# pps-lab/rofl-project-code

Measured on AMD Instinct MI355X. Metric: range-proof elements/sec (create+verify), d=25k 32-bit, higher is better.
Workload: dtype u32x8 (255-bit integer field)

## Files before the change

### rofl_project_code_amd/csrc/host_prover.hpp

```cpp
#pragma once

void tr_append_point(Merlin &t, const char *label, const ge5 &p, uint8_t *enc_out) {
    uint8_t e[32]; h51::encode(e, p); t.append(label, e, 32); if (enc_out) memcpy(enc_out, e, 32);
}
void fill_pow2(sc *tab, sc base_mont, int count) { tab[0] = base_mont; for (int i = 1; i < count; i++) tab[i] = sc_montmul(tab[i - 1], tab[i - 1]); }

sc sum_partials(const sc *p, size_t count, size_t stride, size_t which) {
    sc acc = sc_zero();
    for (size_t i = 0; i < count; i++) acc = sc_add(acc, p[i * stride + which]);
    return acc;
}

struct ChunkNonce { int mode; NonceSeed seed; const uint8_t *d_stream; u64 stream_scalars, base; };
void prove_chunks(Ctx &C, const char *label, size_t P, size_t n, size_t m, const u64 *d_vshift, const sc *d_blind,
                  const std::vector<ChunkNonce> &nonces, const uint8_t *h_V , uint8_t *const *proofs_out,
                  hipEvent_t v_ready = nullptr ) {
    size_t N = n * m; unsigned lgN = lg2u(N);
    static const bool ptrace = knob("ROFL_TRACE") && atoi(knob("ROFL_TRACE")) >= 2;
    double pt0 = now_ms(), ptl = pt0;
    auto mark = [&](const char *what, long a = -1) {
        if (!ptrace) return;
        double t = now_ms(); fprintf(stderr, "[rofl-trace lane=%p] %-14s %6ld  +%.3f ms  (t=%.3f)\n", (void *)&C, what, a, t - ptl, t - pt0); ptl = t;
    };
    size_t plen = 32 * (9 + 2 * (size_t)lgN);
    GensPin gens = get_gens(C, n, m);
    niels *tbl = gens.tbl();
    const niels *wtab = gens.wtab();
    ChunkParams *h_cp = C.h_cp.as<ChunkParams>(P);
    ChunkParams *d_cp = C.cp.as<ChunkParams>(P);
    memset(h_cp, 0, sizeof(ChunkParams) * P);
    u64 per = (u64)m * (2 * n + 4);
    for (size_t c = 0; c < P; c++) {
        h_cp[c].nonce_base = nonces[c].base; h_cp[c].nonce_mode = nonces[c].mode; h_cp[c].nonce_seed = nonces[c].seed;
        h_cp[c].nonce_stream = nonces[c].d_stream; h_cp[c].nonce_stream_scalars = nonces[c].stream_scalars;
    }
    HIPCHK(hipMemcpyAsync(d_cp, h_cp, sizeof(ChunkParams) * P, hipMemcpyHostToDevice, C.stream));
    sc *sL = C.sL.as<sc>(P * N), *sR = C.sR.as<sc>(P * N), *party = C.party.as<sc>(P * 4 * m), *Scanon = C.Scanon.as<sc>(P * 2 * N);
    ROFL_LAUNCH(k_nonce_expand, grid1(per / 2 + 1, (u32)P), dim3(TPB), 0, C.stream, (u32)n, (u32)m, d_cp, sL, sR, party, Scanon);
    if (!C.stream2) HIPCHK(hipStreamCreateWithFlags(&C.stream2, hipStreamNonBlocking));
    if (!C.ev_a) { HIPCHK(hipEventCreateWithFlags(&C.ev_a, hipEventDisableTiming)); HIPCHK(hipEventCreateWithFlags(&C.ev_a0, hipEventDisableTiming)); }
    HIPCHK(hipEventRecord(C.ev_a0, C.stream));
    HIPCHK(hipStreamWaitEvent(C.stream2, C.ev_a0, 0));
    ge *partial = C.partial.as<ge>(P * m);
    ROFL_LAUNCH(k_bitcommit, grid1(m, (u32)P), dim3(TPB), 0, C.stream2, (u32)n, (u32)m, d_vshift, tbl, partial);
    u32 nblkA = (u32)std::min<size_t>(16, (m + TPB - 1) / TPB);
    ge *partial2 = C.partial2.as<ge>(P * nblkA);
    ROFL_LAUNCH(k_point_sum, dim3(nblkA, (u32)P), dim3(TPB), TPB * sizeof(ge), C.stream2, partial, (u32)m, partial2);
    ge *h_A = C.h_part.as<ge>(P * nblkA);
    HIPCHK(hipMemcpyAsync(h_A, partial2, sizeof(ge) * P * nblkA, hipMemcpyDeviceToHost, C.stream2));
    HIPCHK(hipEventRecord(C.ev_a, C.stream2));
    u32 nblkS = (u32)std::min<size_t>(16, (m + TPB - 1) / TPB);
    sc *scpart = C.scpart.as<sc>(P * 64 * 3);
    PowTabs *d_pt = C.powtabs.as<PowTabs>(P);
    ROFL_LAUNCH(k_party_sums, dim3(nblkS, (u32)P), dim3(TPB), 0, C.stream, (u32)m, 0, d_cp, (const PowTabs *)d_pt, party, d_blind, scpart);
    sc *h_sc = C.h_misc2.as<sc>(P * 64 * 3);
    HIPCHK(hipMemcpyAsync(h_sc, scpart, sizeof(sc) * P * nblkS * 3, hipMemcpyDeviceToHost, C.stream));
    std::vector<MsmProb> probs(P); std::vector<ge5> res;
    for (size_t c = 0; c < P; c++) probs[c] = MsmProb{tbl, Scanon + c * 2 * N};
    C.tm.t.msm_terms += P * 2 * N;
    mark("setup");
    std::vector<Merlin> tr; tr.reserve(P);
    std::vector<sc> a_bl(P), s_bl(P), y(P), z(P), zz(P), x(P), w(P);
    for (size_t c = 0; c < P; c++) tr.emplace_back(label, strlen(label));
    {
        MsmOpt mo; mo.tag = 99; if (wtab) { gens.fb_for(P, &mo.fb_wtab, &mo.fb_c); mo.fb_stride = 2 * N; }
        mo.overlap = [&]() {
            double t0 = now_ms();
            if (v_ready) HIPCHK(hipEventSynchronize(v_ready));
            C.pool->run(P, [&](size_t c) {
                Merlin &t = tr[c];
                t.append("dom-sep", (const uint8_t *)"rangeproof v1", 13);
                t.append_u64("n", n); t.append_u64("m", m);
                t.append32_run('V', h_V + c * m * 32, m);
            });
            C.tm.t.host_ms += now_ms() - t0;
        };
        msm_run(C, probs, 2 * N, res, mo);
    }
    mark("msm S");
    HIPCHK(hipEventSynchronize(C.ev_a));

    double th = now_ms();
    C.pool->run(P, [&](size_t c) {
        uint8_t *o = proofs_out[c];
        Merlin &t = tr[c];
        a_bl[c] = h_canon(sum_partials(h_sc + c * nblkS * 3, nblkS, 3, 0));
        s_bl[c] = h_canon(sum_partials(h_sc + c * nblkS * 3, nblkS, 3, 1));
        ge5 A = h_fixed_mul(C.ht.Bb5, a_bl[c]);
        for (u32 k = 0; k < nblkA; k++) A = h51::gadd(A, h51::from_ge(h_A[c * nblkA + k]));
        ge5 S = h51::gadd(res[c], h_fixed_mul(C.ht.Bb5, s_bl[c]));
        tr_append_point(t, "A", A, o); tr_append_point(t, "S", S, o + 32);
        y[c] = t.challenge_scalar("y"); z[c] = t.challenge_scalar("z");
        zz[c] = h_mul(z[c], z[c]);
        ChunkParams &cp = h_cp[c];
        cp.y = h_mont(y[c]); cp.z = h_mont(z[c]); cp.zz = h_mont(zz[c]);
        cp.yinv = h_mont(h_inv(y[c]));
        fill_pow2(cp.ypow2, cp.y, MAX_LG); fill_pow2(cp.yinvpow2, cp.yinv, MAX_LG); fill_pow2(cp.zpow2, cp.z, MAX_LG);
    });
    C.tm.t.host_ms += now_ms() - th;
    mark("y z host");
    HIPCHK(hipMemcpyAsync(d_cp, h_cp, sizeof(ChunkParams) * P, hipMemcpyHostToDevice, C.stream));
    u32 nblkT = (u32)std::min<size_t>(std::max<size_t>(64, std::min<size_t>(256, 2048 / P)), (N + TPB - 1) / TPB);
    sc *tpart = C.tmp_out.as<sc>(P * 256 * 3);
    ROFL_LAUNCH(k_pow_tables, dim3((4 * PT_L * PT_E + TPB - 1) / TPB, (u32)P), dim3(TPB), 0, C.stream, d_cp, d_pt, lgN, 0);
    ROFL_LAUNCH(k_poly_t, dim3(nblkT, (u32)P), dim3(TPB), 0, C.stream, (u32)n, (u32)m, d_cp, (const PowTabs *)d_pt, d_vshift, sL, sR, C.d_two_pow, tpart);
    ROFL_LAUNCH(k_party_sums, dim3(nblkS, (u32)P), dim3(TPB), 0, C.stream, (u32)m, 1, d_cp, (const PowTabs *)d_pt, party, d_blind, scpart);
    sc *h_t = C.h_part.as<sc>(P * 256 * 3);
    HIPCHK(hipMemcpyAsync(h_t, tpart, sizeof(sc) * P * nblkT * 3, hipMemcpyDeviceToHost, C.stream));
    HIPCHK(hipMemcpyAsync(h_sc, scpart, sizeof(sc) * P * nblkS * 3, hipMemcpyDeviceToHost, C.stream));
    C.sync();
    mark("t kernels");
    th = now_ms();
    C.pool->run(P, [&](size_t c) {
        uint8_t *o = proofs_out[c];
        Merlin &t = tr[c];
        sc t0 = h_canon(sum_partials(h_t + c * nblkT * 3, nblkT, 3, 0));
        sc t1 = h_canon(sum_partials(h_t + c * nblkT * 3, nblkT, 3, 1));
        sc t2 = h_canon(sum_partials(h_t + c * nblkT * 3, nblkT, 3, 2));
        sc t1_bl = h_canon(sum_partials(h_sc + c * nblkS * 3, nblkS, 3, 0));
        sc t2_bl = h_canon(sum_partials(h_sc + c * nblkS * 3, nblkS, 3, 1));
        sc zvbl = h_canon(sum_partials(h_sc + c * nblkS * 3, nblkS, 3, 2));
        ge5 T1 = h51::gadd(h_fixed_mul(C.ht.B5, t1), h_fixed_mul(C.ht.Bb5, t1_bl));
        ge5 T2 = h51::gadd(h_fixed_mul(C.ht.B5, t2), h_fixed_mul(C.ht.Bb5, t2_bl));
        tr_append_point(t, "T_1", T1, o + 64); tr_append_point(t, "T_2", T2, o + 96);
        x[c] = t.challenge_scalar("x");
        sc xx = h_mul(x[c], x[c]);
        sc t_x = sc_add(sc_add(t0, h_mul(t1, x[c])), h_mul(t2, xx));
        sc t_x_bl = sc_add(sc_add(zvbl, h_mul(t1_bl, x[c])), h_mul(t2_bl, xx));
        sc e_bl = sc_add(a_bl[c], h_mul(s_bl[c], x[c]));
        t.append_scalar("t_x", t_x); t.append_scalar("t_x_blinding", t_x_bl); t.append_scalar("e_blinding", e_bl);
        sc_tobytes(o + 128, t_x); sc_tobytes(o + 160, t_x_bl); sc_tobytes(o + 192, e_bl);
        w[c] = t.challenge_scalar("w");
        h_cp[c].x = h_mont(x[c]);
        h_cp[c].gscale = sc_one_mont(); h_cp[c].hscale = sc_one_mont();
        t.append("dom-sep", (const uint8_t *)"ipp v1", 6);
        t.append_u64("n", N);
    });
    C.tm.t.host_ms += now_ms() - th;
    mark("T x host");
    HIPCHK(hipMemcpyAsync(d_cp, h_cp, sizeof(ChunkParams) * P, hipMemcpyHostToDevice, C.stream));
    sc *a = C.a.as<sc>(P * N), *b = C.b.as<sc>(P * N), *yinvpow = C.yinv.as<sc>(P * N);
    const u32 lr_first_blocks = (u32)std::min<size_t>(256, (N / 2 + TPB - 1) / TPB);
    ROFL_LAUNCH(k_lr_first, dim3(lr_first_blocks, (u32)P), dim3(TPB), 0, C.stream, (u32)n, (u32)m, d_cp, (const PowTabs *)d_pt, d_vshift, sL, sR, C.d_two_pow, a, b, yinvpow,
                       C.SL.as<sc>(P * 2 * N), C.h_ip.dev<sc>(P * 256 * 2));
    mark("poly/T/x");

    size_t n_g = N; unsigned r = 0;
    std::vector<const niels *> cur(P, tbl);
    std::vector<std::vector<sc>> pu(P), pui(P);
    std::vector<sc> gscale(P, sc_one_mont()), hscale(P, sc_one_mont());
    int gsel = 0; bool first_level = true;
    auto stab = [&](size_t c, u32 h, sc &g, sc &hh) {
        g = sc_one_mont(); hh = sc_one_mont();
        for (unsigned q = 0; q < r; q++) {
            bool bit = (h >> (r - 1 - q)) & 1;
            g = sc_montmul(g, bit ? pu[c][q] : pui[c][q]);
            hh = sc_montmul(hh, bit ? pui[c][q] : pu[c][q]);
        }
    };
    sc *h_round = C.h_round.as<sc>(2 * P);
    sc *a2 = C.a2.as<sc>(P * N), *b2 = C.b2.as<sc>(P * N);
    bool just_materialised = false;
    sc *ptab[2] = {C.ptab[0].as<sc>(P * 2 * N), C.ptab[1].as<sc>(P * 2 * N)}; int psel = 0;
    std::unique_ptr<std::atomic<int>[]> lr_done(new std::atomic<int>[P]);
    sc *ip_dev = C.ipdev.as<sc>(P * 256 * 2);
    niels *d_q = C.qpts.as<niels>(P);
    {
        niels *h_q = C.h_q.as<niels>(P);
        C.pool->run(P, [&](size_t c) { h_q[c] = h51::to_niels32(h_fixed_mul(C.ht.B5, w[c])); });
        HIPCHK(hipMemcpyAsync(d_q, h_q, sizeof(niels) * P, hipMemcpyHostToDevice, C.stream));
    }
    bool ip_included = false, pts_pending = false;
    std::vector<ge5> cq;
    for (unsigned round = 0; round < lgN; round++) {
        size_t n_k = n_g >> r, nh = n_k / 2;
        sc *SL = C.SL.as<sc>(P * 2 * n_g);
        u32 nblkI = lr_first_blocks;
        sc *h_ip = C.h_ip.as<sc>(P * 256 * 2);
        if (round > 0) {
            nblkI = (u32)std::min<size_t>(256, std::max<size_t>(1, (n_g + TPB - 1) / TPB));
            int use_new = just_materialised ? 0 : 1;
            ROFL_LAUNCH(k_ipp_round, dim3(nblkI, (u32)P), dim3(TPB), 0, C.stream, (u32)n_g, (u32)n_k, use_new ? r - 1 : 0u, use_new, d_cp,
                               (const sc *)C.h_round.dev<sc>(2 * P), (const sc *)a, (const sc *)b, a2, b2, N, yinvpow, N, SL, C.h_ip.dev<sc>(P * 256 * 2),
                               (const sc *)ptab[psel], ptab[psel ^ 1], N, n_k == 2 ? C.h_abfin.dev<sc>(4 * P) : (sc *)nullptr, ip_dev);
            std::swap(a, a2); std::swap(b, b2); psel ^= 1;
        }
        just_materialised = false;
        if (!C.ev_ip) HIPCHK(hipEventCreateWithFlags(&C.ev_ip, hipEventDisableTiming));
        HIPCHK(hipEventRecord(C.ev_ip, C.stream));
        std::vector<MsmProb> pr(2 * P);
        for (size_t c = 0; c < P; c++) { pr[2 * c] = MsmProb{cur[c], SL + c * 2 * n_g}; pr[2 * c + 1] = MsmProb{cur[c], SL + c * 2 * n_g}; }
        C.tm.t.msm_terms += P * 2 * n_g;
        MsmOpt mo;
        mo.lr_nh = (u32)nh; mo.lr_ng = (u32)n_g;
        mo.tag = 100 + round;
        if (pts_pending) { mo.pts_ready = C.ev_norm; pts_pending = false; }
        if (round > 0) { mo.ip_dev = ip_dev; mo.ip_nblk = nblkI; mo.qpts = d_q; mo.ip_included = &ip_included; }
        if (first_level && wtab) { gens.fb_for(2 * P, &mo.fb_wtab, &mo.fb_c); mo.fb_stride = 2 * N; }
        for (size_t c = 0; c < P; c++) lr_done[c].store(0);
        bool cq_ready = false;
        auto cq_of = [&](size_t p) { sc cx = h_canon(sum_partials(h_ip + (p >> 1) * nblkI * 2, nblkI, 2, p & 1)); return h_fixed_mul(C.ht.B5, h_mul(cx, w[p >> 1])); };
        mo.overlap = [&]() {
            if (ip_included) return;
            C.wait_event(C.ev_ip);
            cq.resize(2 * P);
            C.pool->run(2 * P, [&](size_t p) { cq[p] = cq_of(p); });
            cq_ready = true;
        };
        auto with_cq = [&](size_t p) { return ip_included ? res[p] : h51::gadd(res[p], cq_ready ? cq[p] : cq_of(p)); };
        mo.post = [&](size_t p) {
            size_t c = p >> 1; int side = (int)(p & 1);
            uint8_t *o = proofs_out[c] + 7 * 32 + 64 * round;
            h51::encode(o + 32 * side, with_cq(p));
            if (lr_done[c].fetch_add(1) != 1) return;
            tr[c].append("L", o, 32); tr[c].append("R", o + 32, 32);
            sc u = tr[c].challenge_scalar("u");
            sc um = h_mont(u), uim = h51::sc_invert_mont_fast(um);
            h_round[2 * c] = um; h_round[2 * c + 1] = uim;
            h_cp[c].pend_u[pu[c].size()] = um; h_cp[c].pend_ui[pu[c].size()] = uim;
            pu[c].push_back(um); pui[c].push_back(uim);
        };
        mo.post8 = [&](size_t p0, int cnt) {
            ge5 pts[8];
            for (int l = 0; l < 8; l++) {
                if (l >= cnt) { pts[l] = h51::identity(); continue; }
                pts[l] = with_cq(p0 + (size_t)l);
            }
            uint8_t enc[8][32];
            h8::encode8(enc, pts);
            const int nch = cnt / 2;
            sc um[4], pre[4];
            for (int k = 0; k < nch; k++) {
                size_t c = (p0 >> 1) + (size_t)k;
                uint8_t *o = proofs_out[c] + 7 * 32 + 64 * round;
                memcpy(o, enc[2 * k], 32); memcpy(o + 32, enc[2 * k + 1], 32);
                tr[c].append("L", o, 32); tr[c].append("R", o + 32, 32);
                um[k] = h_mont(tr[c].challenge_scalar("u"));
                pre[k] = k ? sc_montmul(pre[k - 1], um[k]) : um[k];
            }
            sc uim[4];
            if (nch && !sc_iszero(h_canon(pre[nch - 1]))) {
                sc inv = h51::sc_invert_mont_fast(pre[nch - 1]);
                for (int k = nch - 1; k >= 1; k--) { uim[k] = sc_montmul(inv, pre[k - 1]); inv = sc_montmul(inv, um[k]); }
                uim[0] = inv;
            } else
                for (int k = 0; k < nch; k++) uim[k] = h51::sc_invert_mont_fast(um[k]);
            for (int k = 0; k < nch; k++) {
                size_t c = (p0 >> 1) + (size_t)k;
                h_round[2 * c] = um[k]; h_round[2 * c + 1] = uim[k];
                h_cp[c].pend_u[pu[c].size()] = um[k]; h_cp[c].pend_ui[pu[c].size()] = uim[k];
                pu[c].push_back(um[k]); pui[c].push_back(uim[k]);
            }
        };
        msm_run(C, pr, 2 * n_g, res, mo);
        mark("round msm", (long)(2 * n_g));
        bool last = (round + 1 == lgN);
        r++;
        unsigned t_now = first_level ? (unsigned)C.fold_t1 : (unsigned)C.fold_t;
        size_t n_after = n_g >> r;
        bool fold_pays = n_after >= C.fold_min || (n_after >= 64 && 2 * P * n_after >= 8 * C.fold_min);
        if (!last && r >= t_now && fold_pays) {
            size_t n_new = n_g >> r; u32 nsrc = 1u << r;
            bool use_tab = first_level && C.fold_tab;
            FoldTabCfg fc = gens.fc();
            size_t dstride = use_tab ? (size_t)fc.np * FOLD_TAB_DIGITS : 256;
            th = now_ms();
            const size_t dbytes = use_tab ? 2 : 1;
            int8_t *h_dig = C.h_fdig.as<int8_t>(2 * P * nsrc * dstride * dbytes);
            int16_t *h_dig16 = reinterpret_cast<int16_t *>(h_dig);
            memset(h_dig, 0, 2 * P * nsrc * dstride * dbytes);
            FoldProb *h_fp = C.h_fprob.as<FoldProb>(2 * P);
            niels *gnew = C.gbuf[gsel].as<niels>(P * 2 * n_new);
            std::vector<int> topc(P, 0);
            C.pool->run(P, [&](size_t c) {
                int top = 0;
                sc yn = sc_one_mont();
                sc ystep = sc_one_mont();
                { size_t e = n_new; int bidx = 0; while (e) { if (e & 1) ystep = sc_montmul(ystep, h_cp[c].yinvpow2[bidx]); e >>= 1; bidx++; } }
                sc g0, h0; stab(c, 0, g0, h0);
                sc gall, hall; stab(c, nsrc - 1, gall, hall);
                for (u32 h = 1; h < nsrc; h++) {
                    sc g, hh; stab(c, h, g, hh);
                    yn = sc_montmul(yn, ystep);
                    hh = sc_montmul(hh, yn);
                    g = sc_montmul(g, gall); hh = sc_montmul(hh, hall);
                    sc gc = h_canon(g), hc = h_canon(hh);
                    if (use_tab) {
                        for (u32 pc = 0; pc < fc.np; pc++) {
                            auto piece = [&](const sc &s) {
                                u32 bit0 = pc * fc.pb; u64 lo = (u64)s.v[bit0 / 32] | ((bit0 / 32 + 1 < 8) ? (u64)s.v[bit0 / 32 + 1] << 32 : 0);
                                lo >>= (bit0 % 32);
                                return fc.pb == 64 ? lo : (lo & (((u64)1 << fc.pb) - 1));
                            };
                            int t1 = wnaf_u64(h_dig16 + (((2 * c) * nsrc + h) * fc.np + pc) * FOLD_TAB_DIGITS, piece(gc), fc.w);
                            int t2 = wnaf_u64(h_dig16 + (((2 * c + 1) * nsrc + h) * fc.np + pc) * FOLD_TAB_DIGITS, piece(hc), fc.w);
// ... 117 lines not shown
```

### rofl_project_code_amd/csrc/kernels.hpp

```cpp
#pragma once
#include <type_traits>
#include "fe32.hpp"
#include "fe26.hpp"
#include "quad26.hpp"
#include "keccak.hpp"

namespace rofl {

#define TPB 256

#ifndef ROFL_KGROUP
#define ROFL_KGROUP 0
#endif
#define ROFL_KG(g) (ROFL_KGROUP == 0 || ROFL_KGROUP == (g))

typedef unsigned int v4u __attribute__((ext_vector_type(4)));
typedef __attribute__((address_space(1))) v4u g_uint4;
__device__ __forceinline__ niels gload_niels(const niels *p) {
    niels r;
    const g_uint4 *s = (const g_uint4 *)p;
    v4u *d = reinterpret_cast<v4u *>(&r);
#pragma unroll
    for (int i = 0; i < 6; i++) d[i] = s[i];
    return r;
// ... 285 lines not shown
    if (v != v) st |= 2;
    if (st) { atomicOr(status, st); vshift[i] = 0; return; }
    double x = fabs((double)v) * (double)(1ULL << fp_frac);
    double lim = ldexp(1.0, (int)fp_bits);
    u64 maxbits = fp_bits >= 64 ? ~0ULL : ((1ULL << fp_bits) - 1);
    u64 k;
    if (x >= lim) k = maxbits;
    else { double r = rint(x); k = (r >= lim) ? maxbits : (u64)r; }
    u64 off = 1ULL << (prove_range - 1);
    u64 lowbits;
    if (v < 0.0f) {
        if (off >= k) lowbits = off - k;
        else {
            u64 l_lo = ((u64)SC_L1 << 32) | SC_L0;
            lowbits = l_lo - (k - off);
        }
    } else lowbits = k + off;
    vshift[i] = lowbits & maxbits;
}
#endif

__device__ __forceinline__ gd fixed_base_mul_acc(gd acc, const niels *tab, const sc &k, int nwin) {
    int carry = 0;
    for (int i = 0; i < nwin; i++) {
        int v = (int)((k.v[i >> 2] >> ((i & 3) * 8)) & 255) + carry;
        carry = (v + 128) >> 8;
        int dgt = v - (carry << 8);
        int ad = dgt < 0 ? -dgt : dgt;
        if (ad) acc = gd_madd(acc, load_nd(&tab[i * 128 + ad - 1]), dgt < 0);
    }
    if (carry && nwin < 32) acc = gd_madd(acc, load_nd(&tab[nwin * 128 + 0]), false);
    return acc;
}
#if ROFL_KG(4)
__global__ void __launch_bounds__(TPB) k_commit(u32 count, const u64 *v64, const sc *v256_canon, const sc *blind_canon ,
                         const niels *tabB, const niels *tabBb, const niels *shift ,
                         uint8_t *V_out , uint8_t *C_out , u32 c_count, u32 c_period) {
    u32 j = blockIdx.x * blockDim.x + threadIdx.x;
    if (j >= count) return;
    gd acc = gd_identity();
    if (v64) { sc v = sc_from_u64(v64[j]); acc = fixed_base_mul_acc(acc, tabB, v, 8); }
    else { sc v = load_sc_reduced(&v256_canon[j]); acc = fixed_base_mul_acc(acc, tabB, v, 32); }
    if (blind_canon) { sc r = load_sc_reduced(&blind_canon[j]); acc = fixed_base_mul_acc(acc, tabBb, r, 32); }
    if (V_out) gd_ristretto_encode(V_out + (size_t)j * 32, acc);
    if (C_out && (j % c_period) < c_count) {
        gd cpt = shift ? gd_madd(acc, load_nd(shift), false) : acc;
        gd_ristretto_encode(C_out + (size_t)j * 32, cpt);
    }
}
#endif

#if ROFL_KG(4)
__global__ void __launch_bounds__(TPB) k_bitcommit(u32 n, u32 m, const u64 *vshift , const niels *tbl, ge *partial ) {
    u32 c = blockIdx.y;
    u32 j = blockIdx.x * blockDim.x + threadIdx.x;
    if (j >= m) return;
    size_t N = (size_t)n * m;
    u64 v = vshift[(size_t)c * m + j];
    gd acc = gd_identity();
    for (u32 i = 0; i < n; i++) {
        bool bit = (v >> i) & 1;
        const niels *p = bit ? &tbl[(size_t)j * n + i] : &tbl[N + (size_t)j * n + i];
        acc = gd_madd(acc, gload_nd(p), !bit);
    }
    store_gd(&partial[(size_t)c * m + j], acc);
}
#endif

#if ROFL_KG(4)
__global__ void __launch_bounds__(TPB) k_point_sum(const ge *in, u32 n, ge *out) {
    extern __shared__ __align__(16) unsigned char smem[];
    ge *lds = reinterpret_cast<ge *>(smem);
    u32 p = blockIdx.y, t = threadIdx.x;
    const ge *src = in + (size_t)p * n;
    ge acc = ge_identity();
    for (u32 i = blockIdx.x * blockDim.x + t; i < n; i += gridDim.x * blockDim.x) acc = ge_add(acc, load_ge(&src[i]));
    lds[t] = acc;
    __syncthreads();
    for (u32 s = blockDim.x / 2; s > 0; s >>= 1) {
        if (t < s) lds[t] = ge_add(lds[t], lds[t + s]);
        __syncthreads();
    }
    if (t == 0) store_ge(&out[(size_t)p * gridDim.x + blockIdx.x], lds[0]);
}
#endif

#if ROFL_KG(4)
__global__ void __launch_bounds__(TPB) k_niels_sum(const niels *in, u32 n, size_t stride, ge *out) {
    extern __shared__ __align__(16) unsigned char smem[];
    ge *lds = reinterpret_cast<ge *>(smem);
    u32 t = threadIdx.x;
    const niels *src = in + (size_t)blockIdx.y * stride;
    gd acc = gd_identity();
    for (u32 i = blockIdx.x * blockDim.x + t; i < n; i += gridDim.x * blockDim.x) acc = gd_madd(acc, load_nd(&src[i]), false);
    lds[t] = gd_pack(acc);
    __syncthreads();
    for (u32 s = blockDim.x / 2; s > 0; s >>= 1) {
        if (t < s) lds[t] = ge_add(lds[t], lds[t + s]);
        __syncthreads();
    }
    if (t == 0) store_ge(&out[(size_t)blockIdx.y * gridDim.x + blockIdx.x], lds[0]);
}
#endif

#if ROFL_KG(4)
__global__ void __launch_bounds__(TPB) k_decode_sum(const uint8_t *in, u32 n, u32 stride, ge *out, u32 *status) {
    extern __shared__ __align__(16) unsigned char smem[];
    ge *lds = reinterpret_cast<ge *>(smem);
    u32 t = threadIdx.x;
    gd gacc = gd_identity();
    for (u32 i = blockIdx.x * blockDim.x + t; i < n; i += gridDim.x * blockDim.x) {
        __align__(16) uint8_t b[32];
        const uint8_t *s = in + (size_t)i * stride;
        for (int q = 0; q < 32; q++) b[q] = s[q];
        gd p;
        if (!gd_ristretto_decode(p, b)) { atomicOr(status, 4u); p = gd_identity(); }
        gacc = gd_add(gacc, p);
    }
    lds[t] = gd_pack(gacc);
    __syncthreads();
    for (u32 s = blockDim.x / 2; s > 0; s >>= 1) {
        if (t < s) lds[t] = ge_add(lds[t], lds[t + s]);
        __syncthreads();
    }
    if (t == 0) store_ge(&out[blockIdx.x], lds[0]);
}
#endif

#if ROFL_KG(4)
__global__ void __launch_bounds__(TPB) k_party_sums(u32 m, int phase, const ChunkParams *cp, const PowTabs *pt, const sc *party, const sc *blind_canon , sc *out) {
    __shared__ sc lds[TPB * 3];
    u32 c = blockIdx.y;
    sc v[3] = {sc_zero(), sc_zero(), sc_zero()};
    for (u32 j = blockIdx.x * blockDim.x + threadIdx.x; j < m; j += gridDim.x * blockDim.x) {
        if (phase == 0) {
            v[0] = sc_add(v[0], load_sc(&party[((size_t)c * 4 + 0) * m + j]));
            v[1] = sc_add(v[1], load_sc(&party[((size_t)c * 4 + 1) * m + j]));
        } else {
            v[0] = sc_add(v[0], load_sc(&party[((size_t)c * 4 + 2) * m + j]));
            v[1] = sc_add(v[1], load_sc(&party[((size_t)c * 4 + 3) * m + j]));
            sc zj = sc_montmul(cp[c].zz, pt_pow(pt[c].z, cp[c].zpow2, j));
            sc bl = sc_to_mont(load_sc(&blind_canon[(size_t)c * m + j]));
            v[2] = sc_add(v[2], sc_montmul(zj, bl));
        }
    }
    block_sum_sc<3>(v, lds);
    if (threadIdx.x == 0) {
#pragma unroll
        for (int k = 0; k < 3; k++) store_sc(&out[((size_t)c * gridDim.x + blockIdx.x) * 3 + k], v[k]);
    }
}
#endif

__device__ __forceinline__ void slot_vectors(const ChunkParams &P, const PowTabs &T, u32 n, u32 k, u64 v, const sc &sR,
                                             sc &l0, sc &r0, sc &r1, const sc *two_pow) {
    u32 j = k / n, i = k % n;
    bool bit = (v >> i) & 1;
    sc one = sc_one_mont();
    sc aL = bit ? one : sc_zero();
    sc aR = bit ? sc_zero() : sc_neg(one);
    sc yk = pt_pow(T.y, P.ypow2, k);
    l0 = sc_sub(aL, P.z);
    sc zj2 = sc_montmul(sc_montmul(P.zz, pt_pow(T.z, P.zpow2, j)), two_pow[i]);
    r0 = sc_add(sc_montmul(yk, sc_add(aR, P.z)), zj2);
    r1 = sc_montmul(yk, sR);
}
#if ROFL_KG(4)
__global__ void __launch_bounds__(TPB) k_poly_t(u32 n, u32 m, const ChunkParams *cp, const PowTabs *pt, const u64 *vshift, const sc *sL, const sc *sR,
                         const sc *two_pow, sc *out) {
    __shared__ sc lds[TPB * 3];
    u32 c = blockIdx.y;
    size_t N = (size_t)n * m;
    sc v[3] = {sc_zero(), sc_zero(), sc_zero()};
    for (u32 k = blockIdx.x * blockDim.x + threadIdx.x; k < N; k += gridDim.x * blockDim.x) {
        sc l0, r0, r1;
        sc l1 = load_sc(&sL[c * N + k]);
        slot_vectors(cp[c], pt[c], n, k, vshift[(size_t)c * m + k / n], load_sc(&sR[c * N + k]), l0, r0, r1, two_pow);
        v[0] = sc_add(v[0], sc_montmul(l0, r0));
        v[1] = sc_add(v[1], sc_add(sc_montmul(l0, r1), sc_montmul(l1, r0)));
        v[2] = sc_add(v[2], sc_montmul(l1, r1));
    }
    block_sum_sc<3>(v, lds);
    if (threadIdx.x == 0) {
#pragma unroll
        for (int k = 0; k < 3; k++) store_sc(&out[((size_t)c * gridDim.x + blockIdx.x) * 3 + k], v[k]);
    }
}
#endif

#if ROFL_KG(4)
__global__ void __launch_bounds__(TPB, 3) k_lr_first(u32 n, u32 m, const ChunkParams *cp, const PowTabs *pt, const u64 *vshift, const sc *sL, const sc *sR,
                           const sc *two_pow, sc *a, sc *b, sc *yinvpow, sc *SL, sc *ip_out) {
    __shared__ sc lds[TPB * 2];
    const u32 c = blockIdx.y;
    const size_t N = (size_t)n * m;
    const u32 nh = (u32)(N / 2);
    const sc sG = load_sc(&cp[c].gscale), sH0 = load_sc(&cp[c].hscale), x = cp[c].x;
    sc *sl = SL + (size_t)c * 2 * N;
    sc v[2] = {sc_zero(), sc_zero()};
    for (u32 i = blockIdx.x * blockDim.x + threadIdx.x; i < nh; i += gridDim.x * blockDim.x) {
        sc a0 = sc_zero(), b0 = a0, y0 = a0, a1 = a0, b1 = a0, y1 = a0;
#pragma unroll 1
        for (int s = 0; s < 2; s++) {
            const u32 k = s ? nh + i : i;
            sc l0, r0, r1;
            sc l1 = load_sc(&sL[c * N + k]);
            slot_vectors(cp[c], pt[c], n, k, vshift[(size_t)c * m + k / n], load_sc(&sR[c * N + k]), l0, r0, r1, two_pow);
            sc ao = sc_add(l0, sc_montmul(l1, x));
            sc bo = sc_add(r0, sc_montmul(r1, x));
            sc yo = pt_pow(pt[c].yinv, cp[c].yinvpow2, k);
            store_sc(&a[c * N + k], ao); store_sc(&b[c * N + k], bo); store_sc(&yinvpow[c * N + k], yo);
            if (s == 0) { a0 = ao; b0 = bo; y0 = yo; } else { a1 = ao; b1 = bo; y1 = yo; }
        }
        store_sc(&sl[i], sc_from_mont(sc_montmul(a1, sG)));
        store_sc(&sl[N + i], sc_from_mont(sc_montmul(b1, sc_montmul(sH0, y0))));
        store_sc(&sl[nh + i], sc_from_mont(sc_montmul(a0, sG)));
        store_sc(&sl[N + nh + i], sc_from_mont(sc_montmul(b0, sc_montmul(sH0, y1))));
        v[0] = sc_add(v[0], sc_montmul(a0, b1));
        v[1] = sc_add(v[1], sc_montmul(a1, b0));
    }
    block_sum_sc<2>(v, lds);
    if (threadIdx.x == 0) {
        store_sc(&ip_out[((size_t)c * gridDim.x + blockIdx.x) * 2 + 0], v[0]);
        store_sc(&ip_out[((size_t)c * gridDim.x + blockIdx.x) * 2 + 1], v[1]);
    }
}
#endif


#if ROFL_KG(4)
__global__ void __launch_bounds__(TPB) k_ipp_round(u32 n_g, u32 n_k, u32 r_prev, int use_new, ChunkParams *cp, const sc *round_ch, const sc *a_in, const sc *b_in,
                                                   sc *a_out, sc *b_out, size_t ab_stride, const sc *yinvpow, size_t y_stride, sc *SL, sc *ip_out,
                                                   const sc *ptab_in, sc *ptab_out, size_t ptab_stride, sc *ab_host, sc *ip_dev) {
    __shared__ sc lds[TPB * 2];
    __shared__ sc s_u[2];
    u32 c = blockIdx.y;
    if (threadIdx.x == 0) { s_u[0] = load_sc(&round_ch[2 * c]); s_u[1] = load_sc(&round_ch[2 * c + 1]); }
    __syncthreads();
    const sc u = s_u[0], ui = s_u[1];
    if (use_new && blockIdx.x == 0 && threadIdx.x == 0) { store_sc(&cp[c].pend_u[r_prev], u); store_sc(&cp[c].pend_ui[r_prev], ui); }
    const sc *ai = a_in + c * ab_stride, *bi = b_in + c * ab_stride;
    sc *ao = a_out + c * ab_stride, *bo = b_out + c * ab_stride;
    const u32 nh = n_k / 2;
    const sc gs = sc_from_mont(load_sc(&cp[c].gscale)), hs = sc_from_mont(load_sc(&cp[c].hscale));
    sc *sl = SL + (size_t)c * 2 * n_g;
    sc v[2] = {sc_zero(), sc_zero()};
    auto fold2 = [](const sc &x, const sc &cu, const sc &y, const sc &cv) {
        u32 w[17];
#pragma unroll
        for (int q = 0; q < 17; q++) w[q] = 0;
        sc_mac_wide(w, x, cu); sc_mac_wide(w, y, cv);
        return sc_redc_wide(w);
    };
    for (u32 j = blockIdx.x * blockDim.x + threadIdx.x; j < n_g; j += gridDim.x * blockDim.x) {
        u32 h = j / n_k, i = j % n_k;
        bool lo = i < nh; u32 ii = lo ? nh + i : i - nh;
        sc af = fold2(load_sc(&ai[ii]), u, load_sc(&ai[n_k + ii]), ui);
        sc bf = fold2(load_sc(&bi[ii]), ui, load_sc(&bi[n_k + ii]), u);
        u32 hp = use_new ? h >> 1 : h;
        sc tG = r_prev ? load_sc(&ptab_in[(size_t)c * 2 * ptab_stride + hp]) : gs;
        sc tH = r_prev ? load_sc(&ptab_in[(size_t)c * 2 * ptab_stride + ptab_stride + hp]) : hs;
        if (use_new) { bool bit = h & 1; tG = sc_montmul(tG, bit ? u : ui); tH = sc_montmul(tH, bit ? ui : u); }
        if (i == 0) { store_sc(&ptab_out[(size_t)c * 2 * ptab_stride + h], tG); store_sc(&ptab_out[(size_t)c * 2 * ptab_stride + ptab_stride + h], tH); }
        const sc sG = tG, sH = sc_montmul(tH, load_sc(&yinvpow[c * y_stride + j]));
        store_sc(&sl[j], sc_montmul(af, sG));
        store_sc(&sl[n_g + j], sc_montmul(bf, sH));
        if (h == 0) {
            store_sc(&ao[ii], af); store_sc(&bo[ii], bf);
            if (ab_host && n_k == 2) { store_sc(&ab_host[c * 4 + ii], af); store_sc(&ab_host[c * 4 + 2 + ii], bf); }
            if (lo) {
                sc al = fold2(load_sc(&ai[i]), u, load_sc(&ai[n_k + i]), ui);
                sc bl = fold2(load_sc(&bi[i]), ui, load_sc(&bi[n_k + i]), u);
                v[0] = sc_add(v[0], sc_montmul(al, bf));
                v[1] = sc_add(v[1], sc_montmul(af, bl));
            }
        }
    }
    block_sum_sc<2>(v, lds);
    if (threadIdx.x == 0) {
        store_sc(&ip_out[((size_t)c * gridDim.x + blockIdx.x) * 2 + 0], v[0]);
        store_sc(&ip_out[((size_t)c * gridDim.x + blockIdx.x) * 2 + 1], v[1]);
        if (ip_dev) {
            store_sc(&ip_dev[((size_t)c * gridDim.x + blockIdx.x) * 2 + 0], v[0]);
            store_sc(&ip_dev[((size_t)c * gridDim.x + blockIdx.x) * 2 + 1], v[1]);
        }
    }
}
#endif

struct FoldProb { const niels *src; niels *dst; };
#define FOLD_MAXSRC 64
#define FOLD_MAXSEG 4
struct FoldSeg { int lo[FOLD_MAXSEG + 1]; };
#if ROFL_KG(2)
__global__ void __launch_bounds__(256, 4) k_fold_gens(u32 n_new, u32 nsrc, FoldSeg seg, const FoldProb *probs, const int8_t *naf , int unit_first) {
    extern __shared__ __align__(16) unsigned char smem[];
    ge *lds = reinterpret_cast<ge *>(smem);
    u32 q = blockIdx.y;
    u32 i = blockIdx.x * 64 + threadIdx.x;
    u32 k = threadIdx.y, K = blockDim.y;
    bool active = i < n_new;
    const niels *src = probs[q].src;
    const int8_t *dg = naf + (size_t)q * nsrc * 256;
    gd acc = gd_identity();
    if (active) {
        int lo = seg.lo[k], hi = seg.lo[k + 1] - 1;
        for (int bit = hi; bit >= lo; bit--) {
            acc = gd_double(acc);
            for (u32 h = unit_first ? 1 : 0; h < nsrc; h++) {
                int d = dg[h * 256 + bit];
                if (d != 0) acc = gd_madd(acc, gload_nd(&src[(size_t)h * n_new + i]), d < 0);
            }
        }
        for (int t = 0; t < lo; t++) acc = gd_double(acc);
    }
    if (K > 1) {
        if (k > 0) lds[(k - 1) * 64 + threadIdx.x] = gd_pack(acc);
        __syncthreads();
        if (k == 0)
            for (u32 s2 = 1; s2 < K; s2++) acc = gd_add(acc, gd_unpack(lds[(s2 - 1) * 64 + threadIdx.x]));
    }
    if (active && k == 0) {
        if (unit_first) acc = gd_madd(acc, gload_nd(&src[i]), false);
        gstore_niels(&probs[q].dst[i], gd_to_niels(acc));
    }
}
#endif

#if ROFL_KG(2)
__global__ void __launch_bounds__(256, 2) k_fold_gens4(u32 n_new, FoldSeg seg, const FoldProb *probs, const int8_t *naf ) {
    extern __shared__ __align__(16) unsigned char smem[];
    ge *lds = reinterpret_cast<ge *>(smem);
    u32 q = blockIdx.y;
    u32 i = blockIdx.x * 64 + threadIdx.x;
    u32 k = threadIdx.y, K = blockDim.y;
    bool active = i < n_new;
    const niels *src = probs[q].src;
    const int8_t *dg = naf + (size_t)q * 4 * 256;
    gd acc = gd_identity();
    if (active) {
        const nd s1 = gload_nd(&src[(size_t)1 * n_new + i]), s2 = gload_nd(&src[(size_t)2 * n_new + i]), s3 = gload_nd(&src[(size_t)3 * n_new + i]);
        int lo = seg.lo[k], hi = seg.lo[k + 1] - 1;
        for (int bit = hi; bit >= lo; bit--) {
            acc = gd_double(acc);
            int d1 = dg[256 + bit], d2 = dg[512 + bit], d3 = dg[768 + bit];
            if (d1 != 0) acc = gd_madd(acc, s1, d1 < 0);
            if (d2 != 0) acc = gd_madd(acc, s2, d2 < 0);
            if (d3 != 0) acc = gd_madd(acc, s3, d3 < 0);
        }
        for (int t = 0; t < lo; t++) acc = gd_double(acc);
    }
    if (K > 1) {
        if (k > 0) lds[(k - 1) * 64 + threadIdx.x] = gd_pack(acc);
        __syncthreads();
        if (k == 0)
            for (u32 s2i = 1; s2i < K; s2i++) acc = gd_add(acc, gd_unpack(lds[(s2i - 1) * 64 + threadIdx.x]));
    }
    if (active && k == 0) {
        acc = gd_madd(acc, gload_nd(&src[i]), false);
        gstore_niels(&probs[q].dst[i], gd_to_niels(acc));
    }
}
#endif

#define FOLD_TAB_DIGITS 72
struct FoldWProb { const niels *src; niels *dst; u32 tab_off, ev_off, n_ev, seg_start[FOLD_MAXSEG]; };
#define FOLD_EV(bit, h, e, neg) ((u32)(bit) | ((u32)(h) << 9) | ((u32)(e) << 15) | ((u32)(neg) << 27))
#if ROFL_KG(2)
__device__ __forceinline__ void fold_w_body(u32 n_new, const FoldSeg &seg, const FoldWProb *probs, const u32 *events, const niels *tab, size_t tstride, ge *ext_out) {
    extern __shared__ __align__(16) unsigned char smem[];
    ge *lds = reinterpret_cast<ge *>(smem);
    const u32 q = blockIdx.y;
    const u32 i = blockIdx.x * 64 + threadIdx.x;
    const u32 k = threadIdx.y, K = blockDim.y;
    const bool active = i < n_new;
    const niels *src = probs[q].src;
    const u32 *ev = events + probs[q].ev_off;
    gd acc = gd_identity();
    if (active) {
        const niels *tb = tab + probs[q].tab_off;
        auto operand = [&](u32 w) { const u32 h = (w >> 9) & 63u, e = (w >> 15) & 4095u;
                                    const niels *p = e ? tb + (size_t)(e - 1) * tstride : src;
                                    return gload_nd(&p[(size_t)h * n_new + i]); };
        const int lo = seg.lo[k];
        int pos = seg.lo[k + 1];
        u32 j = probs[q].seg_start[k];
        const u32 jend = k == 0 ? probs[q].n_ev : probs[q].seg_start[k - 1];
        if (j < jend) {
            u32 w = ev[j];
            nd nxt = operand(w);
            while (j < jend) {
                const nd cur = nxt; const u32 wc = w;
                j++;
                if (j < jend) { w = ev[j]; nxt = operand(w); }
                const int b = (int)(wc & 511u);
                for (; pos > b; pos--) acc = gd_double(acc);
                acc = gd_madd(acc, cur, (wc >> 27) & 1u);
            }
        }
        for (; pos > lo; pos--) acc = gd_double(acc);
        for (int t = 0; t < lo; t++) acc = gd_double(acc);
    }
    if (K > 1) {
        if (k > 0) lds[(k - 1) * 64 + threadIdx.x] = gd_pack(acc);
        __syncthreads();
        if (k == 0)
            for (u32 s2 = 1; s2 < K; s2++) acc = gd_add(acc, gd_unpack(lds[(s2 - 1) * 64 + threadIdx.x]));
    }
    if (active && k == 0) {
        acc = gd_madd(acc, gload_nd(&src[i]), false);
        if (ext_out) store_gd(&ext_out[(size_t)q * n_new + i], acc);
        else gstore_niels(&probs[q].dst[i], gd_to_niels(acc));
    }
}
__global__ void __launch_bounds__(256, 2) k_fold_gens_w(u32 n_new, FoldSeg seg, const FoldWProb *probs, const u32 *events, const niels *tab, size_t tstride, ge *ext_out) {
    fold_w_body(n_new, seg, probs, events, tab, tstride, ext_out);
}
#endif

#define NB_BATCH 8
#if ROFL_KG(2)
__global__ void __launch_bounds__(TPB) k_niels_batch(u32 count, const ge *ext, niels *out) {
    const u32 t = blockIdx.x * blockDim.x + threadIdx.x;
    const size_t i0 = (size_t)t * NB_BATCH;
    if (i0 >= count) return;
    const u32 nb = (u32)min((size_t)NB_BATCH, (size_t)count - i0);
    fe pre[NB_BATCH];
    fd run = fd_unpack(reinterpret_cast<const fe *>(&ext[i0])[2]);
// ... 1554 lines not shown
```

Before: 1.148 million.

## Process slot runs incrementally and hoist per-block pending scales in IPP round

```diff
diff --git a/rofl_project_code_amd/csrc/host_prover.hpp b/rofl_project_code_amd/csrc/host_prover.hpp
--- a/rofl_project_code_amd/csrc/host_prover.hpp
+++ b/rofl_project_code_amd/csrc/host_prover.hpp
@@ -100,7 +100,7 @@
     C.tm.t.host_ms += now_ms() - th;
     mark("y z host");
     HIPCHK(hipMemcpyAsync(d_cp, h_cp, sizeof(ChunkParams) * P, hipMemcpyHostToDevice, C.stream));
-    u32 nblkT = (u32)std::min<size_t>(std::max<size_t>(64, std::min<size_t>(256, 2048 / P)), (N + TPB - 1) / TPB);
+    u32 nblkT = (u32)std::min<size_t>(std::max<size_t>(64, std::min<size_t>(256, 2048 / P)), (N / SLOT_RUN + TPB - 1) / TPB);
     sc *tpart = C.tmp_out.as<sc>(P * 256 * 3);
     ROFL_LAUNCH(k_pow_tables, dim3((4 * PT_L * PT_E + TPB - 1) / TPB, (u32)P), dim3(TPB), 0, C.stream, d_cp, d_pt, lgN, 0);
     ROFL_LAUNCH(k_poly_t, dim3(nblkT, (u32)P), dim3(TPB), 0, C.stream, (u32)n, (u32)m, d_cp, (const PowTabs *)d_pt, d_vshift, sL, sR, C.d_two_pow, tpart);
@@ -140,7 +140,7 @@
     mark("T x host");
     HIPCHK(hipMemcpyAsync(d_cp, h_cp, sizeof(ChunkParams) * P, hipMemcpyHostToDevice, C.stream));
     sc *a = C.a.as<sc>(P * N), *b = C.b.as<sc>(P * N), *yinvpow = C.yinv.as<sc>(P * N);
-    const u32 lr_first_blocks = (u32)std::min<size_t>(256, (N / 2 + TPB - 1) / TPB);
+    const u32 lr_first_blocks = (u32)std::min<size_t>(256, (N / 2 / SLOT_RUN + TPB - 1) / TPB);
     ROFL_LAUNCH(k_lr_first, dim3(lr_first_blocks, (u32)P), dim3(TPB), 0, C.stream, (u32)n, (u32)m, d_cp, (const PowTabs *)d_pt, d_vshift, sL, sR, C.d_two_pow, a, b, yinvpow,
                        C.SL.as<sc>(P * 2 * N), C.h_ip.dev<sc>(P * 256 * 2));
     mark("poly/T/x");
diff --git a/rofl_project_code_amd/csrc/kernels.hpp b/rofl_project_code_amd/csrc/kernels.hpp
--- a/rofl_project_code_amd/csrc/kernels.hpp
+++ b/rofl_project_code_amd/csrc/kernels.hpp
@@ -461,18 +461,25 @@
 }
 #endif
 
-__device__ __forceinline__ void slot_vectors(const ChunkParams &P, const PowTabs &T, u32 n, u32 k, u64 v, const sc &sR,
-                                             sc &l0, sc &r0, sc &r1, const sc *two_pow) {
-    u32 j = k / n, i = k % n;
-    bool bit = (v >> i) & 1;
-    sc one = sc_one_mont();
-    sc aL = bit ? one : sc_zero();
-    sc aR = bit ? sc_zero() : sc_neg(one);
-    sc yk = pt_pow(T.y, P.ypow2, k);
-    l0 = sc_sub(aL, P.z);
-    sc zj2 = sc_montmul(sc_montmul(P.zz, pt_pow(T.z, P.zpow2, j)), two_pow[i]);
-    r0 = sc_add(sc_montmul(yk, sc_add(aR, P.z)), zj2);
+#define SLOT_RUN 4
+struct SlotConsts { sc y, z, zm1, l0_set, l0_clr; };
+__device__ __forceinline__ SlotConsts slot_consts(const ChunkParams &P) {
+    SlotConsts K;
+    K.y = P.y; K.z = P.z;
+    K.l0_clr = sc_neg(P.z);
+    K.l0_set = sc_add(sc_one_mont(), K.l0_clr);
+    K.zm1 = sc_neg(K.l0_set);
+    return K;
+}
+__device__ __forceinline__ sc slot_run_zj2(const ChunkParams &P, const PowTabs &T, u32 n, u32 k0, const sc *two_pow) {
+    return sc_montmul(sc_montmul(P.zz, pt_pow(T.z, P.zpow2, k0 / n)), two_pow[k0 % n]);
+}
+__device__ __forceinline__ void slot_step(const SlotConsts &K, bool bit, const sc &sR, sc &yk, sc &zj2, sc &l0, sc &r0, sc &r1) {
+    l0 = bit ? K.l0_set : K.l0_clr;
+    r0 = sc_add(sc_montmul(yk, bit ? K.z : K.zm1), zj2);
     r1 = sc_montmul(yk, sR);
+    yk = sc_montmul(yk, K.y);
+    zj2 = sc_add(zj2, zj2);
 }
 #if ROFL_KG(4)
 __global__ void __launch_bounds__(TPB) k_poly_t(u32 n, u32 m, const ChunkParams *cp, const PowTabs *pt, const u64 *vshift, const sc *sL, const sc *sR,
@@ -480,15 +487,29 @@
     __shared__ sc lds[TPB * 3];
     u32 c = blockIdx.y;
     size_t N = (size_t)n * m;
+    const u32 runs = (u32)(N / SLOT_RUN);
+    const SlotConsts K = slot_consts(cp[c]);
     sc v[3] = {sc_zero(), sc_zero(), sc_zero()};
-    for (u32 k = blockIdx.x * blockDim.x + threadIdx.x; k < N; k += gridDim.x * blockDim.x) {
-        sc l0, r0, r1;
-        sc l1 = load_sc(&sL[c * N + k]);
-        slot_vectors(cp[c], pt[c], n, k, vshift[(size_t)c * m + k / n], load_sc(&sR[c * N + k]), l0, r0, r1, two_pow);
-        v[0] = sc_add(v[0], sc_montmul(l0, r0));
-        v[1] = sc_add(v[1], sc_add(sc_montmul(l0, r1), sc_montmul(l1, r0)));
-        v[2] = sc_add(v[2], sc_montmul(l1, r1));
-    }
+    sc r0_all = sc_zero(), r0_set = r0_all, r1_all = r0_all, r1_set = r0_all;
+    for (u32 q = blockIdx.x * blockDim.x + threadIdx.x; q < runs; q += gridDim.x * blockDim.x) {
+        const u32 k0 = q * SLOT_RUN;
+        const u64 bits = vshift[(size_t)c * m + k0 / n] >> (k0 % n);
+        sc yk = pt_pow(pt[c].y, cp[c].ypow2, k0);
+        sc zj2 = slot_run_zj2(cp[c], pt[c], n, k0, two_pow);
+#pragma unroll 1
+        for (u32 s = 0; s < SLOT_RUN; s++) {
+            sc l0, r0, r1;
+            sc l1 = load_sc(&sL[c * N + k0 + s]);
+            const bool bit = (bits >> s) & 1;
+            slot_step(K, bit, load_sc(&sR[c * N + k0 + s]), yk, zj2, l0, r0, r1);
+            r0_all = sc_add(r0_all, r0); r0_set = sc_add(r0_set, bit ? r0 : sc_zero());
+            r1_all = sc_add(r1_all, r1); r1_set = sc_add(r1_set, bit ? r1 : sc_zero());
+            v[1] = sc_add(v[1], sc_montmul(l1, r0));
+            v[2] = sc_add(v[2], sc_montmul(l1, r1));
+        }
+    }
+    v[0] = sc_add(r0_set, sc_montmul(K.l0_clr, r0_all));
+    v[1] = sc_add(v[1], sc_add(r1_set, sc_montmul(K.l0_clr, r1_all)));
     block_sum_sc<3>(v, lds);
     if (threadIdx.x == 0) {
 #pragma unroll
@@ -498,35 +519,45 @@
 #endif
 
 #if ROFL_KG(4)
-__global__ void __launch_bounds__(TPB, 3) k_lr_first(u32 n, u32 m, const ChunkParams *cp, const PowTabs *pt, const u64 *vshift, const sc *sL, const sc *sR,
+__global__ void __launch_bounds__(TPB, 2) k_lr_first(u32 n, u32 m, const ChunkParams *cp, const PowTabs *pt, const u64 *vshift, const sc *sL, const sc *sR,
                            const sc *two_pow, sc *a, sc *b, sc *yinvpow, sc *SL, sc *ip_out) {
     __shared__ sc lds[TPB * 2];
     const u32 c = blockIdx.y;
     const size_t N = (size_t)n * m;
-    const u32 nh = (u32)(N / 2);
-    const sc sG = load_sc(&cp[c].gscale), sH0 = load_sc(&cp[c].hscale), x = cp[c].x;
+    const u32 nh = (u32)(N / 2), lgh = 31 - __clz(nh);
+    const SlotConsts K = slot_consts(cp[c]);
+    const sc x = cp[c].x, yinv = cp[c].yinv;
+    const sc gs = sc_from_mont(load_sc(&cp[c].gscale)), hs = sc_from_mont(load_sc(&cp[c].hscale));
     sc *sl = SL + (size_t)c * 2 * N;
     sc v[2] = {sc_zero(), sc_zero()};
-    for (u32 i = blockIdx.x * blockDim.x + threadIdx.x; i < nh; i += gridDim.x * blockDim.x) {
-        sc a0 = sc_zero(), b0 = a0, y0 = a0, a1 = a0, b1 = a0, y1 = a0;
-#pragma unroll 1
-        for (int s = 0; s < 2; s++) {
-            const u32 k = s ? nh + i : i;
+    for (u32 q = blockIdx.x * blockDim.x + threadIdx.x; q < nh / SLOT_RUN; q += gridDim.x * blockDim.x) {
+        const u32 i0 = q * SLOT_RUN;
+        const u64 bits0 = vshift[(size_t)c * m + i0 / n] >> (i0 % n), bits1 = vshift[(size_t)c * m + (nh + i0) / n] >> ((nh + i0) % n);
+        sc yk0 = pt_pow(pt[c].y, cp[c].ypow2, i0), yo0 = pt_pow(pt[c].yinv, cp[c].yinvpow2, i0);
+        sc yk1 = sc_montmul(yk0, load_sc(&cp[c].ypow2[lgh])), yo1 = sc_montmul(yo0, load_sc(&cp[c].yinvpow2[lgh]));
+        sc zj0 = slot_run_zj2(cp[c], pt[c], n, i0, two_pow), zj1 = slot_run_zj2(cp[c], pt[c], n, nh + i0, two_pow);
+        auto half = [&](u32 k, bool bit, sc &yk, sc &zj2, sc &yo, sc &ao, sc &bo) {
             sc l0, r0, r1;
             sc l1 = load_sc(&sL[c * N + k]);
-            slot_vectors(cp[c], pt[c], n, k, vshift[(size_t)c * m + k / n], load_sc(&sR[c * N + k]), l0, r0, r1, two_pow);
-            sc ao = sc_add(l0, sc_montmul(l1, x));
-            sc bo = sc_add(r0, sc_montmul(r1, x));
-            sc yo = pt_pow(pt[c].yinv, cp[c].yinvpow2, k);
+            slot_step(K, bit, load_sc(&sR[c * N + k]), yk, zj2, l0, r0, r1);
+            ao = sc_add(l0, sc_montmul(l1, x));
+            bo = sc_add(r0, sc_montmul(r1, x));
             store_sc(&a[c * N + k], ao); store_sc(&b[c * N + k], bo); store_sc(&yinvpow[c * N + k], yo);
-            if (s == 0) { a0 = ao; b0 = bo; y0 = yo; } else { a1 = ao; b1 = bo; y1 = yo; }
-        }
-        store_sc(&sl[i], sc_from_mont(sc_montmul(a1, sG)));
-        store_sc(&sl[N + i], sc_from_mont(sc_montmul(b1, sc_montmul(sH0, y0))));
-        store_sc(&sl[nh + i], sc_from_mont(sc_montmul(a0, sG)));
-        store_sc(&sl[N + nh + i], sc_from_mont(sc_montmul(b0, sc_montmul(sH0, y1))));
-        v[0] = sc_add(v[0], sc_montmul(a0, b1));
-        v[1] = sc_add(v[1], sc_montmul(a1, b0));
+        };
+#pragma unroll 1
+        for (u32 s = 0; s < SLOT_RUN; s++) {
+            const u32 i = i0 + s;
+            sc a0, b0, a1, b1;
+            half(i, (bits0 >> s) & 1, yk0, zj0, yo0, a0, b0);
+            half(nh + i, (bits1 >> s) & 1, yk1, zj1, yo1, a1, b1);
+            store_sc(&sl[i], sc_montmul(a1, gs));
+            store_sc(&sl[N + i], sc_montmul(b1, sc_montmul(hs, yo0)));
+            store_sc(&sl[nh + i], sc_montmul(a0, gs));
+            store_sc(&sl[N + nh + i], sc_montmul(b0, sc_montmul(hs, yo1)));
+            v[0] = sc_add(v[0], sc_montmul(a0, b1));
+            v[1] = sc_add(v[1], sc_montmul(a1, b0));
+            yo0 = sc_montmul(yo0, yinv); yo1 = sc_montmul(yo1, yinv);
+        }
     }
     block_sum_sc<2>(v, lds);
     if (threadIdx.x == 0) {
@@ -551,7 +582,6 @@
     const sc *ai = a_in + c * ab_stride, *bi = b_in + c * ab_stride;
     sc *ao = a_out + c * ab_stride, *bo = b_out + c * ab_stride;
     const u32 nh = n_k / 2;
-    const sc gs = sc_from_mont(load_sc(&cp[c].gscale)), hs = sc_from_mont(load_sc(&cp[c].hscale));
     sc *sl = SL + (size_t)c * 2 * n_g;
     sc v[2] = {sc_zero(), sc_zero()};
     auto fold2 = [](const sc &x, const sc &cu, const sc &y, const sc &cv) {
@@ -561,28 +591,46 @@
         sc_mac_wide(w, x, cu); sc_mac_wide(w, y, cv);
         return sc_redc_wide(w);
     };
-    for (u32 j = blockIdx.x * blockDim.x + threadIdx.x; j < n_g; j += gridDim.x * blockDim.x) {
+    auto pending = [&](u32 h, u32 side) {
+        sc t = r_prev ? load_sc(&ptab_in[(size_t)c * 2 * ptab_stride + side * ptab_stride + (use_new ? h >> 1 : h)])
+                      : sc_from_mont(load_sc(side ? &cp[c].hscale : &cp[c].gscale));
+        if (use_new) t = sc_montmul(t, ((h & 1) != side) ? u : ui);
+        return t;
+    };
+    const bool block_h = n_k % TPB == 0;
+    __shared__ sc s_t[2];
+    for (u32 j0 = blockIdx.x * blockDim.x; j0 < n_g; j0 += gridDim.x * blockDim.x) {
+        const u32 j = j0 + threadIdx.x;
+        sc tG, tH;
+        if (block_h) {
+            __syncthreads();
+            if (threadIdx.x < 2) {
+                const u32 h0 = j0 / n_k;
+                sc t = pending(h0, threadIdx.x);
+                s_t[threadIdx.x] = t;
+                if (j0 % n_k == 0) store_sc(&ptab_out[(size_t)c * 2 * ptab_stride + threadIdx.x * ptab_stride + h0], t);
+            }
+            __syncthreads();
+            tG = s_t[0]; tH = s_t[1];
+        }
+        if (j >= n_g) continue;
         u32 h = j / n_k, i = j % n_k;
         bool lo = i < nh; u32 ii = lo ? nh + i : i - nh;
         sc af = fold2(load_sc(&ai[ii]), u, load_sc(&ai[n_k + ii]), ui);
         sc bf = fold2(load_sc(&bi[ii]), ui, load_sc(&bi[n_k + ii]), u);
-        u32 hp = use_new ? h >> 1 : h;
-        sc tG = r_prev ? load_sc(&ptab_in[(size_t)c * 2 * ptab_stride + hp]) : gs;
-        sc tH = r_prev ? load_sc(&ptab_in[(size_t)c * 2 * ptab_stride + ptab_stride + hp]) : hs;
-        if (use_new) { bool bit = h & 1; tG = sc_montmul(tG, bit ? u : ui); tH = sc_montmul(tH, bit ? ui : u); }
-        if (i == 0) { store_sc(&ptab_out[(size_t)c * 2 * ptab_stride + h], tG); store_sc(&ptab_out[(size_t)c * 2 * ptab_stride + ptab_stride + h], tH); }
+        if (!block_h) {
+            tG = pending(h, 0); tH = pending(h, 1);
+            if (i == 0) { store_sc(&ptab_out[(size_t)c * 2 * ptab_stride + h], tG); store_sc(&ptab_out[(size_t)c * 2 * ptab_stride + ptab_stride + h], tH); }
+        }
         const sc sG = tG, sH = sc_montmul(tH, load_sc(&yinvpow[c * y_stride + j]));
         store_sc(&sl[j], sc_montmul(af, sG));
         store_sc(&sl[n_g + j], sc_montmul(bf, sH));
         if (h == 0) {
             store_sc(&ao[ii], af); store_sc(&bo[ii], bf);
             if (ab_host && n_k == 2) { store_sc(&ab_host[c * 4 + ii], af); store_sc(&ab_host[c * 4 + 2 + ii], bf); }
-            if (lo) {
-                sc al = fold2(load_sc(&ai[i]), u, load_sc(&ai[n_k + i]), ui);
-                sc bl = fold2(load_sc(&bi[i]), ui, load_sc(&bi[n_k + i]), u);
-                v[0] = sc_add(v[0], sc_montmul(al, bf));
-                v[1] = sc_add(v[1], sc_montmul(af, bl));
-            }
+            sc ax = fold2(load_sc(&ai[i]), u, load_sc(&ai[n_k + i]), ui);
+            sc term = sc_montmul(ax, bf);
+            if (lo) v[0] = sc_add(v[0], term); else v[1] = sc_add(v[1], term);
         }
     }
     block_sum_sc<2>(v, lds);
```

Result: no change. 1.151 million (median of 2 runs) (+0.2%).
